# AhmedKishki/AMP-SPARC-SpatialModulation

Hardware: AMD Instinct MI355X
Metric: detected symbol-vectors/sec, VAMP Nt=256 Nr=512 16-QAM; SER match vs ref (higher is better)
Workload: dtype bf16x3; 1 GPU; cfg4: VAMP Nt=256 Nr=512 Na=8 16QAM batch=4096 iterations<=20 EbN0=8.0 dB, one channel per batch; global_batch=4096, parallelism=epoch-shard x1 (independent epochs, one all-reduce of the error counters)

## Files before the change

amp-sparc-spatialmodulation_amd/csrc/amp_denoise.h:

```cpp
#pragma once

#include <float.h>

#include "amp_common.h"

namespace amp {

#define AMP_LOG2E 1.44269504088896340736f

#ifndef AMP_DEN_EXACT_EXP
#define AMP_DEN_EXACT_EXP 0
#endif
#ifndef AMP_DEN_DIV
#define AMP_DEN_DIV 0
#endif
__device__ __forceinline__ float den_exp(float x, float m) {
#if AMP_DEN_EXACT_EXP
    return (float)exp((double)x - (double)m);
#else
    return __builtin_amdgcn_exp2f((x - m) * AMP_LOG2E);
#endif
}
__device__ __forceinline__ float den_rcp(float z) {
#if AMP_DEN_DIV
// ... 542 lines not shown
        for (int i = 0; i < R; ++i) {
            ax = fmaxf(ax, X[i][u]); nx = fminf(nx, X[i][u]);
            ay = fmaxf(ay, Y[i][u]); ny = fminf(ny, Y[i][u]);
        }
        mx[u] = ax; my[u] = ay;
        lmx[u] = ax + ay;
        smax[u] = group_fmax_c<G>(lmx[u]);
        sabs[u] = group_fmax_c<G>(fmaxf(lmx[u], -(nx + ny)));
    }
    const f2v l2e = f2splat(AMP_LOG2E);
#if AMP_DEN_EXACT_EXP
    f2v f = {den_exp(lmx.x, smax.x), den_exp(lmx.y, smax.y)};
#else
    f2v targ = (lmx - smax) * l2e;
    f2v f = {__builtin_amdgcn_exp2f(targ.x), __builtin_amdgcn_exp2f(targ.y)};
#endif
    f2v er[R], ei[R];
#pragma unroll
    for (int i = 0; i < R; ++i) {
#if AMP_DEN_EXACT_EXP
        er[i] = f2v{den_exp(X[i].x, mx.x), den_exp(X[i].y, mx.y)};
        ei[i] = f2v{den_exp(Y[i].x, my.x), den_exp(Y[i].y, my.y)};
#else
        const f2v xa = (X[i] - mx) * l2e, ya = (Y[i] - my) * l2e;
        er[i] = f2v{__builtin_amdgcn_exp2f(xa.x), __builtin_amdgcn_exp2f(xa.y)};
        ei[i] = f2v{__builtin_amdgcn_exp2f(ya.x), __builtin_amdgcn_exp2f(ya.y)};
#endif
    }
    f2v zt, ar, ai, SI = f2splat(0.f);
    f2v Sr[FULLG ? 1 : R];
    if constexpr (FULLG) {
        f2v sr = f2splat(0.f), si = f2splat(0.f), a = f2splat(0.f), b = f2splat(0.f);
#pragma unroll
        for (int i = 0; i < R; ++i) {
            sr += er[i]; si += ei[i];
            a = f2fma(f2splat(Q.re[i]), er[i], a);
            b = f2fma(f2splat(Q.im[i]), ei[i], b);
        }
        SI = si; Sr[0] = sr;
        zt = (sr * si) * f;
        ar = (a * si) * f;
        ai = (sr * b) * f;
    } else {
        f2v z = f2splat(0.f), a = f2splat(0.f), b = f2splat(0.f), w[R];
#pragma unroll
        for (int j = 0; j < R; ++j) w[j] = f2splat(Q.im[j]) * ei[j];
#pragma unroll
        for (int i = 0; i < R; ++i) {
            f2v si = f2splat(0.f), ti = f2splat(0.f);
#pragma unroll
            for (int j = 0; j < R; ++j) {
                const float cw = grid_cnt<PAT>(i, j);
                if (cw == 1.f) { si += ei[j]; ti += w[j]; }
                else if (cw == 2.f) { si = f2fma(f2splat(2.f), ei[j], si); ti = f2fma(f2splat(2.f), w[j], ti); }
            }
            Sr[i] = si;
            const f2v es = er[i] * si;
            z += es;
            a = f2fma(f2splat(Q.re[i]), es, a);
            b = f2fma(er[i], ti, b);
        }
        zt = z * f;
        ar = a * f;
        ai = b * f;
    }
    float ze[2] = {0.f, 0.f}, zt1[2] = {zt.x, zt.y};
#pragma unroll
    for (int u = 0; u < 2; ++u) group_sum_excl_c<G>(zt1[u], ze[u]);
    const f2v iz = {den_rcp(zt1[0]), den_rcp(zt1[1])};
    const f2v xr = ar * iz, xi = ai * iz;
    f2v var = f2splat(0.f);
    if (kVar) {
        f2v vs;
        if constexpr (FULLG) {
            f2v vr = f2splat(0.f), vi = f2splat(0.f);
#pragma unroll
            for (int i = 0; i < R; ++i) {
                const f2v dr = xr - f2splat(Q.re[i]), di = xi - f2splat(Q.im[i]);
                vr = f2fma(dr * dr, er[i], vr);
                vi = f2fma(di * di, ei[i], vi);
            }
            vs = f2fma(vr, SI, Sr[0] * vi) * f;
        } else {
            f2v d[R];
#pragma unroll
            for (int j = 0; j < R; ++j) {
                const f2v di = xi - f2splat(Q.im[j]);
                d[j] = (di * di) * ei[j];
            }
            f2v acc = f2splat(0.f);
#pragma unroll
            for (int i = 0; i < R; ++i) {
                f2v vi = f2splat(0.f);
#pragma unroll
                for (int j = 0; j < R; ++j) {
                    const float cw = grid_cnt<PAT>(i, j);
                    if (cw == 1.f) vi += d[j];
                    else if (cw == 2.f) vi = f2fma(f2splat(2.f), d[j], vi);
                }
                const f2v dr = xr - f2splat(Q.re[i]);
                acc = f2fma(er[i], f2fma(dr * dr, Sr[i], vi), acc);
            }
            vs = acc * f;
        }
        const f2v zev = {ze[0], ze[1]};
        var = (xr * xr + xi * xi) * (zev * iz) + vs * iz;
    }
    xr_out = xr; xi_out = xi; var_out = var; smax_out = smax; sabs_out = sabs;
}

struct Grid2In {
    f2v rr, ri, vp;
};
template <int G, class P>
__device__ __forceinline__ Grid2In grid2_load(const P& pol, int base) {
    const int lane = threadIdx.x & 63;
    constexpr int gpw = 64 / G;
    const int gid = lane / G, g = lane % G;
    Grid2In in;
#pragma unroll
    for (int u = 0; u < 2; ++u) {
        float rr, ri;
        pol.load_r(base + u * gpw + gid, g, rr, ri);
        in.rr[u] = rr; in.ri[u] = ri;
    }
#pragma unroll
    for (int u = 0; u < 2; ++u) in.vp[u] = pol.load_prev(base + u * gpw + gid, g);
    return in;
}
template <bool kVar, int R, int PAT, int G, class P>
__device__ __forceinline__ void denoise_step_grid2_full(const P& pol, int base, const Grid2In& in, const GridRegs<R>& Q,
                                                        PartAcc& pa, DenStat& S) {
    const int lane = threadIdx.x & 63;
    constexpr int gpw = 64 / G;
    const int gid = lane / G, g = lane % G;
    const f2v it = f2splat(pol.inv);
    const f2v ur = in.rr * it, ui = in.ri * it;
    const int bad = (int)!(fabsf(ur.x) <= FLT_MAX) | (int)!(fabsf(ui.x) <= FLT_MAX) | (int)!(fabsf(ur.y) <= FLT_MAX) |
                    (int)!(fabsf(ui.y) <= FLT_MAX);
    S.st_bad |= bad != 0;
    f2v xr, xi, var, smax, sabs;
    grid2_core<kVar, R, PAT, G>(ur, ui, Q, xr, xi, var, smax, sabs);
    pol.store_xv(base + gid, g, xr.x, xi.x, var.x);
    pol.store_xv(base + gpw + gid, g, xr.y, xi.y, var.y);
#pragma unroll
    for (int u = 0; u < 2; ++u) {
        pol.account(var[u], in.vp[u], pa);
        S.st_abs = nan_max(S.st_abs, sabs[u]);
        S.st_min = nan_min(S.st_min, smax[u]);
        pol.section(base + u * gpw + gid, smax[u], sabs[u]);
    }
}

#ifndef AMP_DEN_PACKED_GRID
#define AMP_DEN_PACKED_GRID 1
#endif

template <int KK>
constexpr int grid_r() { return KK == 4 ? 2 : KK == 16 ? 4 : KK == 64 ? 8 : 0; }

template <bool kVar, int KK, int U, int G, bool PKG = true, bool FAST = false, class P>
__device__ __forceinline__ bool denoise_sections_grid(const P& pol, int nsec, const Const& c, PartAcc& pa, DenWaves dw = DenWaves::block()) {
    constexpr int R = grid_r<KK>();
    if constexpr (R == 0) {
        return false;
    } else {
        const int grid = __builtin_amdgcn_readfirstlane(c.grid), gfull = __builtin_amdgcn_readfirstlane(c.gfull);
        if (grid != R) return false;
        const int wave = dw.wave;
        constexpr int gpw = 64 / G;
        const int nw = dw.nw;
        DenStat S;
        GridRegs<R> Q;
        Q.load(c);
        if (gfull == GRID_FULL) {
            for (int base = wave * gpw * U; base < nsec; base += nw * gpw * U) {
                if constexpr (PKG && U == 2 && AMP_DEN_PACKED_GRID)
                    denoise_step_grid2<kVar, R, GRID_FULL, G>(pol, base, nsec, Q, pa, S);
                else
                    denoise_step_grid<kVar, R, GRID_FULL, U, G>(pol, base, nsec, Q, pa, S);
            }
        } else if constexpr (R == 4) {
            int base = wave * gpw * U;
            if constexpr (FAST && PKG && U == 2 && AMP_DEN_PACKED_GRID) {
                const int step = nw * gpw * 2;
                for (; base + 2 * gpw <= nsec; base += step)
                    denoise_step_grid2_full<kVar, R, GRID_REF16, G>(pol, base, grid2_load<G>(pol, base), Q, pa, S);
            }
            for (; base < nsec; base += nw * gpw * U) {
                if constexpr (PKG && U == 2 && AMP_DEN_PACKED_GRID)
                    denoise_step_grid2<kVar, R, GRID_REF16, G>(pol, base, nsec, Q, pa, S);
                else
                    denoise_step_grid<kVar, R, GRID_REF16, U, G>(pol, base, nsec, Q, pa, S);
            }
        }
        S.fold(pa);
        return true;
    }
}

template <bool kVar, int KK, int U, int G, class P>
__device__ __forceinline__ void denoise_sections_gp(const P& pol, int nsec, const Const& c, PartAcc& pa, DenWaves dw = DenWaves::block()) {
    if (denoise_sections_grid<kVar, KK, U, G>(pol, nsec, c, pa, dw)) return;
    const int wave = dw.wave;
    constexpr int gpw = 64 / G;
    const int nw = dw.nw;
    DenRegs<KK> R;
    R.load(c);
    DenStat S;
    for (int base = wave * gpw * U; base < nsec; base += nw * gpw * U)
        denoise_step_gp<kVar, KK, U, G, false>(pol, base, nsec, R, pa, S);
    S.fold(pa);
}

enum { PK_NONE = 0, PK_ALL = 1, PK_GRID = 2 };

template <bool kVar, int KK, int U, int G, int PK, bool FAST = false, class P>
__device__ __forceinline__ void denoise_sections_sel(const P& pol, int nsec, const Const& c, PartAcc& pa, DenWaves dw = DenWaves::block()) {
    if constexpr (PK == PK_ALL && KK % 2 == 0) {
        denoise_sections_gp<kVar, KK, U, G>(pol, nsec, c, pa, dw);
    } else {
        if (denoise_sections_grid<kVar, KK, U, G, PK == PK_GRID, FAST>(pol, nsec, c, pa, dw)) return;
        denoise_sections_g<kVar, KK, U, G>(pol, nsec, c, pa, dw);
    }
}
template <bool kVar, int KK, int U, int PK = PK_ALL, bool FAST = false, class P>
__device__ __forceinline__ void denoise_sections_u(const P& pol, int nsec, int M, const Const& c, PartAcc& pa, DenWaves dw = DenWaves::block()) {
    switch (M) {
    case 64: denoise_sections_sel<kVar, KK, U, 64, PK, FAST>(pol, nsec, c, pa, dw); break;
    case 32: denoise_sections_sel<kVar, KK, U, 32, PK, FAST>(pol, nsec, c, pa, dw); break;
    case 16: denoise_sections_sel<kVar, KK, U, 16, PK, FAST>(pol, nsec, c, pa, dw); break;
    case 8: denoise_sections_sel<kVar, KK, U, 8, PK, FAST>(pol, nsec, c, pa, dw); break;
    case 4: denoise_sections_sel<kVar, KK, U, 4, PK, FAST>(pol, nsec, c, pa, dw); break;
    case 2: denoise_sections_sel<kVar, KK, U, 2, PK, FAST>(pol, nsec, c, pa, dw); break;
    default: denoise_sections_sel<kVar, KK, U, 1, PK, FAST>(pol, nsec, c, pa, dw); break;
    }
}

template <bool kVar, int KK, int G, class P>
__device__ __forceinline__ void denoise_sections_wide(const P& pol, int nsec, const Const& c, PartAcc& pa, DenWaves dw = DenWaves::block()) {
    static_assert(KK % 8 == 0, "chunks of 8 points");
    if (denoise_sections_grid<kVar, KK, 1, G>(pol, nsec, c, pa, dw)) return;
    const int lane = threadIdx.x & 63, wave = dw.wave;
    constexpr int gpw = 64 / G;
    const int gid = lane / G, g = lane % G;
    const int nw = dw.nw;
    __shared__ float s_cre[KK], s_cim[KK];
    __syncthreads();
    if (threadIdx.x == 0) {
#pragma unroll
        for (int k = 0; k < KK; ++k) { s_cre[k] = kval(c.re[k]); s_cim[k] = kval(c.im[k]); }
    }
    __syncthreads();
    DenStat S;
    for (int base = wave * gpw; base < nsec; base += nw * gpw) {
        const int sec = base + gid;
        const bool act = sec < nsec;
        float rr, ri, it;
        pol.load(act ? sec : nsec - 1, g, rr, ri, it);
        const float ur = rr * it, ui = ri * it;
        if (act) S.st_bad |= !(fabsf(ur) <= FLT_MAX && fabsf(ui) <= FLT_MAX);
        float lmax = -FLT_MAX, lmin = FLT_MAX;
#pragma unroll 1
        for (int k0 = 0; k0 < KK; k0 += 8) {
#pragma unroll
            for (int j = 0; j < 8; ++j) {
                const float x = fmaf(ur, s_cre[k0 + j], ui * s_cim[k0 + j]);
                lmax = fmaxf(lmax, x);
                lmin = fminf(lmin, x);
            }
        }
        const float smax = group_fmax_c<G>(lmax), sabs = group_fmax_c<G>(fmaxf(lmax, -lmin));
        float zm = 0.f, a = 0.f, b = 0.f;
#pragma unroll 1
        for (int k0 = 0; k0 < KK; k0 += 8) {
#pragma unroll
            for (int j = 0; j < 8; ++j) {
                const float cr = s_cre[k0 + j], ci = s_cim[k0 + j];
                const float e = den_exp(fmaf(ur, cr, ui * ci), smax);
                zm += e;
                a = fmaf(cr, e, a);
                b = fmaf(ci, e, b);
            }
        }
        float zt = zm, ze = 0.f;
        group_sum_excl_c<G>(zt, ze);
        const float iz = den_rcp(zt);
        const float xr = a * iz, xi = b * iz;
        float var = 0.f;
        if (kVar) {
            float vs = 0.f;
#pragma unroll 1
            for (int k0 = 0; k0 < KK; k0 += 8) {
#pragma unroll
                for (int j = 0; j < 8; ++j) {
                    const float cr = s_cre[k0 + j], ci = s_cim[k0 + j];
                    const float e = den_exp(fmaf(ur, cr, ui * ci), smax);
                    const float dr = xr - cr, di = xi - ci;
                    vs = fmaf(fmaf(dr, dr, di * di), e, vs);
                }
            }
            var = (xr * xr + xi * xi) * (ze * iz) + vs * iz;
        }
        if (act) {
            pol.store(sec, g, xr, xi, var, pa);
            S.st_abs = nan_max(S.st_abs, sabs);
            S.st_min = nan_min(S.st_min, smax);
            if (g == 0) pol.section(sec, smax, sabs);
        }
    }
    S.fold(pa);
}

template <bool kVar, int KK, class P>
__device__ __forceinline__ void denoise_sections_wide_m(const P& pol, int nsec, int M, const Const& c, PartAcc& pa, DenWaves dw = DenWaves::block()) {
    switch (M) {
    case 64: denoise_sections_wide<kVar, KK, 64>(pol, nsec, c, pa, dw); break;
    case 32: denoise_sections_wide<kVar, KK, 32>(pol, nsec, c, pa, dw); break;
    case 16: denoise_sections_wide<kVar, KK, 16>(pol, nsec, c, pa, dw); break;
    case 8: denoise_sections_wide<kVar, KK, 8>(pol, nsec, c, pa, dw); break;
    case 4: denoise_sections_wide<kVar, KK, 4>(pol, nsec, c, pa, dw); break;
    case 2: denoise_sections_wide<kVar, KK, 2>(pol, nsec, c, pa, dw); break;
    default: denoise_sections_wide<kVar, KK, 1>(pol, nsec, c, pa, dw); break;
    }
}

template <bool kVar, int KK, class P>
__device__ __forceinline__ void denoise_sections(const P& pol, int nsec, int M, const Const& c, PartAcc& pa) {
    if constexpr (KK > 16) {
        denoise_sections_wide_m<kVar, KK>(pol, nsec, M, c, pa);
        return;
    } else {
    if (M <= 64) {
        denoise_sections_u<kVar, KK, 1>(pol, nsec, M, c, pa);
        return;
    }
    const int lane = threadIdx.x & 63, wave = threadIdx.x >> 6;
    const int G = M < 64 ? M : 64;
    const int PPL = M / G;
    const int gpw = 64 / G;
    const int gid = lane / G, g = lane - gid * G;
    const int nw = blockDim.x >> 6;
    for (int base = wave * gpw; base < nsec; base += nw * gpw) {
        const int sec = base + gid;
        const bool act = sec < nsec;
        const int ss = act ? sec : nsec - 1;
        float lmax = -FLT_MAX, lmin = FLT_MAX;
        bool bad = false;
        {
            for (int p = 0; p < PPL; ++p) {
                float rr, ri, it;
                pol.load(ss, g + p * 64, rr, ri, it);
                const float ur = rr * it, ui = ri * it;
                bad |= !(fabsf(ur) <= FLT_MAX && fabsf(ui) <= FLT_MAX);
#pragma unroll
                for (int k = 0; k < KK; ++k) {
                    {
                        const float x = fmaf(ur, c.re[k], ui * c.im[k]);
                        lmax = fmaxf(lmax, x);
                        lmin = fminf(lmin, x);
                    }
                }
            }
            const float smax = group_fmax(lmax, 64);
            double zl = 0.0;
            for (int p = 0; p < PPL; ++p) {
                float rr, ri, it;
                pol.load(ss, g + p * 64, rr, ri, it);
                const float ur = rr * it, ui = ri * it;
                float zm = 0.f;
#pragma unroll
                for (int k = 0; k < KK; ++k)
                    zm += __builtin_amdgcn_exp2f((fmaf(ur, c.re[k], ui * c.im[k]) - smax) * AMP_LOG2E);
                zl += (double)zm;
            }
            const double z = group_sum(zl, 64);
            const double iz = 1.0 / z;
            for (int p = 0; p < PPL; ++p) {
                float rr, ri, it;
// ... 131 lines not shown
```

amp-sparc-spatialmodulation_amd/csrc/amp_vamp.h:

```cpp
#pragma once

#include "amp_decide.h"
#include "amp_denoise.h"
#include "amp_gemm.h"
#include "amp_host.h"

namespace amp {

constexpr int RWG = 1024;
constexpr int PBAR_EPOCH = 64;
constexpr int PBAR_WORDS = PBAR_EPOCH + 256;

struct VampK {
    int B, N, n, k, L, M;
    int Bmean;
    int kap0, ncp0, kap1, ncp1, kap2, ncp2, bn2;
    int nblk2, max_iter;
    double noise_var, sparsity;
    const float* Wt0;
    const float* Wt1;
    const float* Wt2;
    const float* s;
    float* s2;
    float* ytil;
// ... 141 lines not shown
    }
    ss = group_sum(ss, 64);
    const float varL = (float)(ss / (double)P.k) * (float)P.noise_var;
    const double eta = (double)P.k / (double)P.N;
    float xtv, s2t32;
    if (first) {
        xtv = (float)eta * varL + (float)((1.0 - eta) * s2t64);
        s2t32 = (float)s2t64;
    } else {
        xtv = (float)eta * varL + (float)(1.0 - eta) * s2t;
        s2t32 = s2t;
    }
    const float alpha = clampf_t(xtv / s2t32, AMP_VAR_RATIO_MIN, 1.0f - AMP_VAR_RATIO_MIN);
    const float sigma2 = clampf_t((alpha / (1.0f - alpha)) * s2t32, AMP_VAR_MIN, AMP_VAR_MAX);
    it.vr = vr;
    it.alpha = alpha;
    it.inv1ma = 1.0f / (1.0f - alpha);
    it.sigma2 = sigma2;
    it.inv_sigma2 = 1.0f / sigma2;
    it.s2t = s2t32;
}

__device__ inline VampIter vamp_first_iter(const VampK& P, float* lds, const S2Lane* sl = nullptr) {
    VampIter it;
    it.stopped = 0; it.T = 0; it.fixed = 0; it.fixed_all = 0; it.G = 0.0;
    it.pad1[0] = it.pad1[1] = it.pad1[2] = 0.f;
    it.dxdr_prev = 0.f;
    it.ns_prev = 1.f;
    const double p = P.sparsity;
    vamp_lmmse_scalars(P, true, p * p * (1 - p) + (1 - p) * (1 - p) * p, 0.f, lds, it, sl);
    return it;
}

__device__ inline VampIter vamp_advance(const VampK& P, const VampIter& cur, const PartAcc& pa, int fixed, int t,
                                        float* lds, const S2Lane* sl = nullptr) {
    VampIter nx;
    nx.stopped = 0; nx.T = 0; nx.fixed = fixed; nx.fixed_all = (fixed < 0) ? 1 : 0; nx.G = pa.maxabs;
    nx.pad1[0] = nx.pad1[1] = nx.pad1[2] = 0.f;
    if (pa.notclose == 0) {
        nx = cur;
        nx.stopped = 1;
        nx.T = t + 1;
        nx.fixed = fixed;
    } else {
        const float mean = (float)(pa.sumvar / ((double)P.Bmean * (double)P.N));
        const float dxdr = clampf_t(mean / cur.sigma2, AMP_VAR_RATIO_MIN, 1.0f - AMP_VAR_RATIO_MIN);
        const float ns = 1.0f / (1.0f - dxdr);
        const float s2t = clampf_t((cur.sigma2 * dxdr) * ns, AMP_VAR_MIN, AMP_VAR_MAX);
        nx.dxdr_prev = dxdr;
        nx.ns_prev = ns;
        vamp_lmmse_scalars(P, false, 0.0, s2t, lds, nx, sl);
    }
    return nx;
}

__device__ inline VampIter vamp_advance_head(const VampK& P, const VampIter& cur, const PartAcc& pa, int fixed, int t) {
    VampIter nx;
    nx.stopped = 0; nx.T = 0; nx.fixed = fixed; nx.fixed_all = (fixed < 0) ? 1 : 0; nx.G = pa.maxabs;
    nx.pad1[0] = nx.pad1[1] = nx.pad1[2] = 0.f;
    nx.vr = nx.alpha = nx.inv1ma = nx.sigma2 = nx.inv_sigma2 = 0.f;
    if (pa.notclose == 0) {
        nx = cur;
        nx.stopped = 1;
        nx.T = t + 1;
        nx.fixed = fixed;
    } else {
        const float mean = (float)(pa.sumvar / ((double)P.Bmean * (double)P.N));
        const float dxdr = clampf_t(mean / cur.sigma2, AMP_VAR_RATIO_MIN, 1.0f - AMP_VAR_RATIO_MIN);
        const float ns = 1.0f / (1.0f - dxdr);
        nx.dxdr_prev = dxdr;
        nx.ns_prev = ns;
        nx.s2t = clampf_t((cur.sigma2 * dxdr) * ns, AMP_VAR_MIN, AMP_VAR_MAX);
    }
    return nx;
}

__device__ inline void vamp_advance_tail(const VampK& P, VampIter& it, const S2Lane& sl) {
    const float s2t = it.s2t;
    const float vr = (1.0f / s2t) * (float)P.noise_var;
    const int lane = threadIdx.x & 63;
    float q[4];
#pragma unroll
    for (int j = 0; j < 4; ++j) q[j] = 1.0f / (sl.v[j] + vr);
    double ss = 0.0;
#pragma unroll
    for (int j = 0; j < 4; ++j) ss += (lane + 64 * j < P.k) ? (double)q[j] : 0.0;
    ss = group_sum(ss, 64);
    const float varL = (float)(ss / (double)P.k) * (float)P.noise_var;
    const float xtv = P.etaf * varL + P.ometaf * s2t;
    const float alpha = clampf_t(xtv / s2t, AMP_VAR_RATIO_MIN, 1.0f - AMP_VAR_RATIO_MIN);
    const float sigma2 = clampf_t((alpha / (1.0f - alpha)) * s2t, AMP_VAR_MIN, AMP_VAR_MAX);
    it.vr = vr;
    it.alpha = alpha;
    it.inv1ma = 1.0f / (1.0f - alpha);
    it.sigma2 = sigma2;
    it.inv_sigma2 = 1.0f / sigma2;
}

__device__ inline amp_status vamp_make_status(const VampK& P, const VampIter& cur, const VampIter& nx, int fixed) {
    amp_status s;
    s.T = nx.stopped ? nx.T : P.max_iter;
    s.nan_state = fixed != 0 ? 1 : 0;
    s.stopped = nx.stopped;
    s.gemm = P.x3 + 1;
    s.last_scalar[0] = cur.s2t; s.last_scalar[1] = cur.alpha; s.last_scalar[2] = cur.sigma2;
    s.last_scalar[3] = nx.stopped ? cur.dxdr_prev : nx.dxdr_prev;
    return s;
}

struct PDenoisePolicy {
    const float* r;
    float* x;
    float* vnew;
    const float* vprev;
    float* sm;
    float* sa;
    int ldr, M, lspr, N;
    float inv;
    __device__ __forceinline__ void load(int sec, int m, float& rr, float& ri, float& it) const {
        const int row = sec >> lspr, sj = sec & ((1 << lspr) - 1);
        const float2 v = *reinterpret_cast<const float2*>(r + row * ldr + 2 * (sj * M + m));
        rr = v.x; ri = v.y; it = inv;
    }
    __device__ __forceinline__ void store(int sec, int m, float xr, float xi, float var, PartAcc& pa) const {
        const int row = sec >> lspr, sj = sec & ((1 << lspr) - 1);
        *reinterpret_cast<float2*>(x + row * ldr + 2 * (sj * M + m)) = make_float2(xr, xi);
        const int vo = row * N + sj * M + m;
        vnew[vo] = var;
        pa.sumvar += (double)var;
        pa.notclose += torch_close(var, vprev[vo]) ? 0u : 1u;
    }
    __device__ __forceinline__ void section(int sec, float smax, float sabs) const {
        sm[sec] = smax;
        sa[sec] = sabs;
    }
    __device__ __forceinline__ void load_r(int sec, int m, float& rr, float& ri) const {
        const int row = sec >> lspr, sj = sec & ((1 << lspr) - 1);
        const float2 v = *reinterpret_cast<const float2*>(r + row * ldr + 2 * (sj * M + m));
        rr = v.x; ri = v.y;
    }
    __device__ __forceinline__ float load_prev(int sec, int m) const {
        const int row = sec >> lspr, sj = sec & ((1 << lspr) - 1);
        return vprev[row * N + sj * M + m];
    }
    __device__ __forceinline__ void store_xv(int sec, int m, float xr, float xi, float var) const {
        const int row = sec >> lspr, sj = sec & ((1 << lspr) - 1);
        *reinterpret_cast<float2*>(x + row * ldr + 2 * (sj * M + m)) = make_float2(xr, xi);
        vnew[row * N + sj * M + m] = var;
    }
    __device__ __forceinline__ void account(float var, float vp, PartAcc& pa) const {
        pa.sumvar += (double)var;
        pa.notclose += torch_close(var, vp) ? 0u : 1u;
    }
    float* dbg = nullptr;
};
__device__ __forceinline__ void den_debug(const PDenoisePolicy& p, int sec, int m, float ze, float vs) {
    if (p.dbg) {
        const int row = sec >> p.lspr, sj = sec & ((1 << p.lspr) - 1);
        p.dbg[row * 2 * p.N + sj * p.M + m] = ze;
        p.dbg[row * 2 * p.N + p.N + sj * p.M + m] = vs;
    }
}

constexpr int PBM = 16;

bool vamp_persist_eligible(const amp_dims* d, int k, int ncu, int epochs = 1, int gemm = AMP_GEMM_AUTO);
int vamp_persist_max_epochs(const amp_dims* d, int k, int ncu, int gemm = AMP_GEMM_AUTO);
int vamp_persist_wg_per_cu(const amp_dims* d, int k, int gemm);
int vamp_gemm_select(const amp_dims* d, int k, int gemm);
bool vamp_persist_x3_fits(int N, int k, int L, int K = 0);
bool vamp_persist_ytil_in_kernel(const VampK& P);
bool vamp_persist_ytil_h2(const VampK& P);
int vamp_persist_launch(const VampK& P, const Const64& c64, const DecConst& dc, hipStream_t st, int ncu);
int device_cu_count();
float* debug_dump_ptr();
bool gemm_f32_requested();
bool persist_wg2();

}
```

amp-sparc-spatialmodulation_amd/csrc/amp_vamp_persist.hip:

```cpp
#include <stdlib.h>

#include <algorithm>
#include <mutex>
#include <vector>

#include "amp_vamp_persist_kernel.h"

namespace amp {

__global__ __launch_bounds__(1024) void vamp_decide_fold(const DecWG* w, int n, amp_counts* out) {
    __shared__ DecWG s[16];
    dec_fold_block(w + (size_t)blockIdx.x * n, n, out + blockIdx.x, s);
}

static std::once_flag g_pers_once;
static int g_ncu = 0;

int device_cu_count() {
    std::call_once(g_pers_once, [] {
        int dev = 0;
        if (hipGetDevice(&dev) != hipSuccess || hipDeviceGetAttribute(&g_ncu, hipDeviceAttributeMultiprocessorCount,
                                                                      dev) != hipSuccess)
            g_ncu = 0;
    });
    return g_ncu;
}

bool vamp_persist_ytil_in_kernel(const VampK& P) {
    return P.n == 2 * P.N && PBM * (2 * P.n + 4) <= playout(P.N, P.k, P.L).offV0;
}

bool vamp_persist_ytil_h2(const VampK& P) {
    return P.n == 2 * P.N && P.k == P.N && 2 * PBM * pl_ldx(P.n) <= playout(P.N, P.k, P.L, true).offV0;
}

bool vamp_persist_x3_fits(int N, int k, int L, int K) {
    const size_t fixed = K > 16 ? 5120 : 2048;
    return k == N && N % 64 == 0 && (size_t)playout(N, k, L, true).total * 4 + fixed <= 160 * 1024;
}

bool persist_wg2() {
    static const bool v = [] {
        const char* e = diag_env("AMP_PERSIST_WG2");
        return !(e && e[0] == '0') && !gemm_f32_requested();
    }();
    return v;
}
static bool persist_pair_epochs() {
    static const bool v = [] {
        const char* e = diag_env("AMP_EPOCHS_TWO_PER_CU");
        return e && e[0] == '1';
    }();
    return v;
}
static int persist_wg_cap(int N, int gemm_mode) {
    return (N == 64 && (gemm_mode == 1 || gemm_mode == 2) && persist_wg2() && persist_pair_epochs()) ? 2 : 1;
}

int vamp_persist_wg_per_cu(const amp_dims* d, int k, int gemm) {
    return persist_wg_cap(d->N, vamp_gemm_select(d, k, gemm));
}

int vamp_persist_max_epochs(const amp_dims* d, int k, int ncu, int gemm) {
    const int gemm_mode = vamp_gemm_select(d, k, gemm);
    if (!vamp_persist_shape(d, k) || d->n % 2 != 0 || d->M > 64) return 0;
    if ((size_t)playout(d->N, k, d->L).total * 4 + 2048 > 160 * 1024) return 0;
    const int wpe = cdiv(d->B, PBM);
    if (wpe > ncu) return 0;
    if (d->B % PBM != 0) return 1;
    return std::max(1, persist_wg_cap(d->N, gemm_mode) * ncu / wpe);
}

bool vamp_persist_eligible(const amp_dims* d, int k, int ncu, int epochs, int gemm) {
    if (!vamp_persist_shape(d, k) || d->n % 2 != 0 || d->M > 64) return false;
    if (epochs < 1 || (epochs > 1 && d->B % PBM != 0)) return false;
    if (cdiv(d->B, PBM) > ncu ||
        (long)epochs * cdiv(d->B, PBM) > (long)persist_wg_cap(d->N, vamp_gemm_select(d, k, gemm)) * ncu)
        return false;
    return (size_t)playout(d->N, k, d->L).total * 4 + 2048 <= 160 * 1024;
}

static int persist_dispatch(const VampK& P, const DecConst& dc, hipStream_t st);
int persist_dispatch_x3(const VampK& P, const DecConst& dc, hipStream_t st);
int persist_dispatch_h2(const VampK& P, const DecConst& dc, hipStream_t st);
int persist_dispatch_i8(const VampK& P, const DecConst& dc, hipStream_t st);

static std::mutex g_tm_mu;
static bool g_tm_on = false;
static std::vector<std::pair<hipEvent_t, hipEvent_t>> g_tm_ev;

int vamp_persist_launch(const VampK& P, const Const64& c64, const DecConst& dc, hipStream_t st, int ncu) {
    (void)ncu;
    DecConst d2 = dc;
    static_cast<Const64&>(d2) = c64;
    hipEvent_t te[2] = {nullptr, nullptr};
    {
        std::lock_guard<std::mutex> lk(g_tm_mu);
        if (g_tm_on && hipEventCreate(&te[0]) == hipSuccess && hipEventCreate(&te[1]) == hipSuccess) {
            g_tm_ev.emplace_back(te[0], te[1]);
            (void)hipEventRecord(te[0], st);
        } else {
            te[0] = te[1] = nullptr;
        }
    }
    const int rc = persist_dispatch(P, d2, st);
    if (te[1]) (void)hipEventRecord(te[1], st);
    if (rc || !P.dec_on || P.fold_in) return rc;
    hipLaunchKernelGGL(vamp_decide_fold, dim3(P.E), dim3(256), 0, st, (const DecWG*)P.dwg, P.nwg / P.E, P.counts);
    AMP_LAUNCH_CHECK("vamp_decide_fold");
    return AMP_OK;
}

static int persist_dispatch(const VampK& P, const DecConst& dc, hipStream_t st) {
    if (P.x3 == 3) return persist_dispatch_i8(P, dc, st);
    if (P.x3 == 2) return persist_dispatch_h2(P, dc, st);
    if (P.x3) return persist_dispatch_x3(P, dc, st);
    switch (P.N) {
    case 64: return persist_launch_nt<2, 4, false>(P, dc, st);
    case 128: return persist_launch_nt<4, 4, false>(P, dc, st);
    case 256: return persist_launch_nt<8, 4, false>(P, dc, st);
    default: break;
    }
    set_error("vamp_persist: N = %d not supported", P.N);
    return AMP_E_ARG;
}

}

int amp_debug_persist_timing(int32_t on) {
    std::lock_guard<std::mutex> lk(amp::g_tm_mu);
    amp::g_tm_on = on != 0;
    return AMP_OK;
}

int amp_debug_persist_time(int32_t* n, float* mean_ms) {
    AMP_REQUIRE(n && mean_ms, "amp_debug_persist_time: null output");
    std::lock_guard<std::mutex> lk(amp::g_tm_mu);
    double tot = 0.0;
    int cnt = 0;
    for (auto& e : amp::g_tm_ev) {
        float ms = 0.f;
        if (hipEventSynchronize(e.second) == hipSuccess && hipEventElapsedTime(&ms, e.first, e.second) == hipSuccess) {
            tot += ms;
            ++cnt;
        }
        (void)hipEventDestroy(e.first);
        (void)hipEventDestroy(e.second);
    }
    amp::g_tm_ev.clear();
    *n = cnt;
    *mean_ms = cnt ? (float)(tot / cnt) : 0.f;
    return AMP_OK;
}
```

amp-sparc-spatialmodulation_amd/csrc/amp_vamp_persist_kernel.h:

```cpp
#pragma once

#include <stdlib.h>

#include <type_traits>

#include "amp_decide_fused.h"
#include "amp_persist.h"
#include "amp_vamp.h"

namespace amp {

constexpr int AMP_TRACE_STRIDE = 10;
#ifndef AMP_OCC2_PK
#define AMP_OCC2_PK 0
#endif
#ifndef AMP_KK4_DU
#define AMP_KK4_DU 4
#endif
#ifndef AMP_X3_W8_PIN
#define AMP_X3_W8_PIN 0
#endif
#ifndef AMP_X3_W8_RING
#define AMP_X3_W8_RING 1
#endif
#ifndef AMP_X3_W8_PKGRID
#define AMP_X3_W8_PKGRID 1
#endif
#ifndef AMP_X3_W8_DENFAST
#define AMP_X3_W8_DENFAST 1
#endif
#ifndef AMP_DECIDE_NARROW
#define AMP_DECIDE_NARROW 1
#endif
#ifndef AMP_X3_DU
#define AMP_X3_DU 2
#endif
#ifndef AMP_SCALAR_TAIL
#define AMP_SCALAR_TAIL 1
#endif

struct PLayout {
    int lda, ldr;
    int offA, offR, offX, offV0, offV1, offSM, offSA, offScr, total;
};

__host__ __device__ inline int x3_ldx(int N) { return pl_ldx(N); }
__host__ __device__ inline int x3_plane_floats(int N) { return 6 * 16 * x3_ldx(N) / 2; }

__host__ __device__ inline PLayout playout(int N, int k, int L, bool x3 = false) {
    PLayout y;
    y.lda = (2 * N > 2 * k ? 2 * N : 2 * k) + 4;
    y.ldr = 2 * N + (x3 ? 8 : 4);
    int o = 0;
    y.offA = o; o += (x3 && x3_plane_floats(N) > PBM * y.lda) ? x3_plane_floats(N) : PBM * y.lda;
    y.offR = o; o += PBM * y.ldr;
    y.offX = o; o += PBM * y.ldr;
    y.offV0 = o; o += PBM * N;
    y.offV1 = o; o += PBM * N;
    y.offSM = o; o += PBM * L;
    y.offSA = o; o += PBM * L;
    o = (o + 3) & ~3;
    y.offScr = o; o += 1024;
    y.total = o;
    return y;
}

constexpr int KARG_DC_OFF = karg_second_offset<VampK, DecConst>();

template <int NT, int KK, int NWV, int DU, bool X3, int OCC = 1, bool H2 = false, bool I8 = false>
__global__ __launch_bounds__(64 * NWV, OCC * NWV / 4) void vamp_persist(VampK P_arg, DecConst dc_arg) {
    (void)P_arg;
    (void)dc_arg;
    unsigned long long kbase = karg_base();
    const VampK* Pp = karg_at<VampK>(kbase, 0);
    const DecConst* Dp = karg_at<DecConst>(kbase, KARG_DC_OFF);
#define P (*Pp)
#define dc (*Dp)
    static_assert(!X3 || ((NWV == 4 || (NWV == 8 && !H2 && OCC == 1)) && NT % 2 == 0),
                  "X3: four waves (eight for the bf16x3 two-waves-per-SIMD form), whole complex tiles");
    static_assert(!(H2 && I8) && (!I8 || X3), "I8: a split-precision form of its own");
    constexpr int PKDEN = ((OCC * NWV / 4 == 1) || AMP_OCC2_PK) ? PK_ALL
                          : (NWV == 8 && KK == 16 && AMP_X3_W8_PKGRID) ? PK_GRID : PK_NONE;
    constexpr bool DENFAST = NWV == 8 && OCC == 1 && PKDEN == PK_GRID && AMP_X3_W8_DENFAST;
    constexpr int PWG = 64 * NWV;
    constexpr int NC = X3 ? NT / 2 : 1;
    constexpr int G3 = NT * NWV / 4;
    constexpr int X3R = (NWV == 8) ? AMP_X3_W8_RING : 1;
    constexpr bool X3PIN = NWV == 8 && AMP_X3_W8_PIN;
    constexpr bool X3PF = X3 && !H2 && !I8;
    constexpr int PFT = (NC + 1) / 2;
    constexpr int STAIL = (X3PF && OCC == 1) ? AMP_SCALAR_TAIL : 0;
#define c64 (static_cast<const Const64&>(*Dp))
    extern __shared__ __attribute__((aligned(16))) float lds[];
    __shared__ int s_flag;
    __shared__ double s_d[PWG / 64][4];
    __shared__ float s_hmax[PWG / 64][PBM];
    __shared__ int s_hexp[PBM];
    __shared__ float s_s2[STAIL != 0 ? 256 : 1];
    const PLayout Y = playout(P.N, P.k, P.L, X3);
    float* sA = lds + Y.offA;
    float* sR = lds + Y.offR;
    float* sX = lds + Y.offX;
    float* sM = lds + Y.offSM;
    float* sS = lds + Y.offSA;
    float* scr = lds + Y.offScr;
    const int tid = threadIdx.x, lane = tid & 63, wave = tid >> 6;
    const int wg = blockIdx.x, nwg = gridDim.x;
    const int wgx = wg + P.wg_off, nwx = P.nwg_x;
    const int ep = wgx / P.wpe, wl = wgx - ep * P.wpe, wg0 = ep * P.wpe;
    const int lrow0 = wl * PBM;
    const int row0 = ep * P.B + lrow0 - P.row_off, nrows = min(PBM, P.B - lrow0);
#define ebar (P.pbar + (P.E > 1 ? PBAR_EPOCH + ep : 0))
    const int N = P.N, twoN = 2 * N, twok = 2 * P.k, M = P.M, spr = N / M;
    const float* const sv_ep = P.s + (size_t)ep * P.sch;
#define Wx1 ((const void*)((const char*)P.Wx1 + ep * P.wch))
#define Wx2 ((const void*)((const char*)P.Wx2 + ep * P.wch))
    const int ldr = Y.ldr, lda = Y.lda;
    const int ct0 = wave * NT;
    const int cc0 = wave * NC;
    unsigned short* sP = reinterpret_cast<unsigned short*>(sA);
    const int ldx = x3_ldx(N);
    signed char* sB = reinterpret_cast<signed char*>(sA);
    const int ldb = i8_ldb(N);

    float yt[NT][4], s2c[NT];
#pragma unroll
    for (int t = 0; t < NT; ++t) {
        const int col = X3 ? 2 * (16 * (cc0 + (t < NC ? t : 0)) + (lane & 15)) : 16 * (ct0 + t) + (lane & 15);
        const float sv = sv_ep[col >> 1];
        s2c[t] = sv * sv;
    }
    if (H2 && P.ytil_in_kernel) {
      if constexpr (H2) {
        constexpr int IPY = NT / 2;
        const int n = P.n, ldy = pl_ldx(n);
        const int row = tid % PBM;
        float re[IPY][8], im[IPY][8];
        float m = 0.f;
#pragma unroll
        for (int i = 0; i < IPY; ++i) {
            const int e = tid + i * PWG;
            const int j0 = 8 * (e / PBM);
#pragma unroll
            for (int h = 0; h < 4; ++h) {
                float4 v = *reinterpret_cast<const float4*>(P.y + (size_t)(row0 + max(min(row, nrows - 1), 0)) * 2 * n + 2 * j0 + 4 * h);
                if (!(row < nrows)) v = make_float4(0.f, 0.f, 0.f, 0.f);
                re[i][2 * h] = v.x; im[i][2 * h] = v.y; re[i][2 * h + 1] = v.z; im[i][2 * h + 1] = v.w;
            }
#pragma unroll
            for (int h = 0; h < 8; ++h) m = fmaxf(m, fmaxf(fabsf(re[i][h]), fabsf(im[i][h])));
        }
        m = fmaxf(m, __shfl_xor(m, 16));
        m = fmaxf(m, __shfl_xor(m, 32));
        if (lane < PBM) s_hmax[wave][lane] = m;
        __syncthreads();
        float mr = s_hmax[0][row];
#pragma unroll
        for (int w = 1; w < PWG / 64; ++w) mr = fmaxf(mr, s_hmax[w][row]);
        const int ex = h2_row_exp(mr);
        if (tid < PBM) s_hexp[tid] = ex;
#pragma unroll
        for (int i = 0; i < IPY; ++i) {
            const int e = tid + i * PWG;
#pragma unroll
            for (int h = 0; h < 8; ++h) {
                re[i][h] = __builtin_amdgcn_ldexpf(re[i][h], ex);
                im[i][h] = __builtin_amdgcn_ldexpf(im[i][h], ex);
            }
            h2_store8(sP, ldy, row, 8 * (e / PBM), re[i], im[i]);
        }
        __syncthreads();
        f32x4 yr[NC], yi[NC];
        gemm_h2<NC, 2 * G3>(sP, ldy, P.Wq0, cc0, yr, yi);
#pragma unroll
        for (int r = 0; r < 4; ++r) {
            const float sc = __builtin_amdgcn_ldexpf(1.0f, -(s_hexp[4 * (lane >> 4) + r] + YH2_EX));
#pragma unroll
            for (int t = 0; t < NC; ++t) {
                yt[2 * t][r] = yr[t][r] * sc;
                yt[2 * t + 1][r] = yi[t][r] * sc;
            }
        }
        __syncthreads();
      }
    } else if (X3) {
      if constexpr (!I8) {
#pragma unroll
        for (int t = 0; t < NC; ++t) {
            const int o = 16 * (cc0 + t) + (lane & 15);
#pragma unroll
            for (int r = 0; r < 4; ++r) {
                const int row = 4 * (lane >> 4) + r;
                const bool in = row < nrows;
                const size_t yo = (size_t)(row0 + max(min(row, nrows - 1), 0)) * twok + 2 * o;
                const float a = P.ytil[yo], b = P.ytil[yo + 1];
                yt[2 * t][r] = in ? a : 0.f;
                yt[2 * t + 1][r] = in ? b : 0.f;
            }
        }
      }
    } else if (P.ytil_in_kernel) {
        const int ldy = 4 * N + 4;
        for (int e = tid; e < PBM * N; e += PWG) {
            const int row = e / N, c4 = 4 * (e - row * N);
            float4 v = *reinterpret_cast<const float4*>(P.y + (size_t)(row0 + max(min(row, nrows - 1), 0)) * 4 * N + c4);
            if (!(row < nrows)) v = make_float4(0.f, 0.f, 0.f, 0.f);
            *reinterpret_cast<float4*>(lds + row * ldy + c4) = v;
        }
        __syncthreads();
        f32x4 acc[NT];
        gemm16<NT, 2 * NT * NWV>(lds, ldy, P.Wq0, ct0, acc);
#pragma unroll
        for (int t = 0; t < NT; ++t)
#pragma unroll
            for (int r = 0; r < 4; ++r) yt[t][r] = acc[t][r];
        __syncthreads();
    } else {
#pragma unroll
        for (int t = 0; t < NT; ++t) {
            const int col = 16 * (ct0 + t) + (lane & 15);
#pragma unroll
            for (int r = 0; r < 4; ++r) {
                const int row = 4 * (lane >> 4) + r;
                const float yv = P.ytil[(size_t)(row0 + max(min(row, nrows - 1), 0)) * twok + col];
                yt[t][r] = (row < nrows) ? yv : 0.f;
            }
        }
    }
    VampIter cur;
    {
        const S2Lane s2l = s2_lane(P, sv_ep);
        cur = vamp_first_iter(P, scr, &s2l);
        if constexpr (STAIL != 0) {
            if (wave == 0) {
#pragma unroll
                for (int j = 0; j < 4; ++j) s_s2[lane + 64 * j] = s2l.v[j];
// ... 553 lines not shown
```

Baseline: 6.084 million symbol-vectors/s.

## Add paired-lane grid denoise path with vectorized loads/stores for 16-QAM

Adds a new denoiser fast path for the 16-QAM grid case with G=32 and eight waves. Each lane now handles two adjacent symbols of one section, so r/x can be read and written as float4 and the variances as float2, and the per-section max reduction needs fewer cross-lane steps. The variance sum is carried in a lane-permuted double accumulator using permlane32_swap and bpermute, so the reduction order matches the old per-lane layout. A host check is added that rejects LDS layouts whose rows are not 16-byte aligned. The risks are extra permute instructions and possible small changes in floating-point ordering.

```diff
diff --git a/amp-sparc-spatialmodulation_amd/csrc/amp_denoise.h b/amp-sparc-spatialmodulation_amd/csrc/amp_denoise.h
--- a/amp-sparc-spatialmodulation_amd/csrc/amp_denoise.h
+++ b/amp-sparc-spatialmodulation_amd/csrc/amp_denoise.h
@@ -718,14 +718,212 @@
     }
 }
 
+template <bool kVar, int R, int PAT>
+__device__ __forceinline__ void grid2_pair_core(const f2v ur, const f2v ui, const GridRegs<R>& Q, f2v& xr_out, f2v& xi_out,
+                                                f2v& var_out, float& smax_out, float& sabs_out) {
+    constexpr bool FULLG = PAT == GRID_FULL;
+    f2v X[R], Y[R];
+#pragma unroll
+    for (int i = 0; i < R; ++i) {
+        X[i] = ur * f2splat(Q.re[i]);
+        Y[i] = ui * f2splat(Q.im[i]);
+    }
+    f2v mx, my, lmx, lab;
+#pragma unroll
+    for (int u = 0; u < 2; ++u) {
+        float ax = -FLT_MAX, nx = FLT_MAX, ay = -FLT_MAX, ny = FLT_MAX;
+#pragma unroll
+        for (int i = 0; i < R; ++i) {
+            ax = fmaxf(ax, X[i][u]); nx = fminf(nx, X[i][u]);
+            ay = fmaxf(ay, Y[i][u]); ny = fminf(ny, Y[i][u]);
+        }
+        mx[u] = ax; my[u] = ay;
+        lmx[u] = ax + ay;
+        lab[u] = fmaxf(lmx[u], -(nx + ny));
+    }
+    int kmax = max(fkey(lmx.x), fkey(lmx.y)), kabs = max(fkey(lab.x), fkey(lab.y));
+    kmax = imax_step<1>(kmax); kabs = imax_step<1>(kabs);
+    kmax = imax_step<2>(kmax); kabs = imax_step<2>(kabs);
+    kmax = imax_step<4>(kmax); kabs = imax_step<4>(kabs);
+    kmax = imax_step<8>(kmax); kabs = imax_step<8>(kabs);
+    const float smax1 = funkey(kmax), sabs1 = funkey(kabs);
+    const f2v smax = f2splat(smax1);
+    const f2v l2e = f2splat(AMP_LOG2E);
+#if AMP_DEN_EXACT_EXP
+    f2v f = {den_exp(lmx.x, smax.x), den_exp(lmx.y, smax.y)};
+#else
+    f2v targ = (lmx - smax) * l2e;
+    f2v f = {__builtin_amdgcn_exp2f(targ.x), __builtin_amdgcn_exp2f(targ.y)};
+#endif
+    f2v er[R], ei[R];
+#pragma unroll
+    for (int i = 0; i < R; ++i) {
+#if AMP_DEN_EXACT_EXP
+        er[i] = f2v{den_exp(X[i].x, mx.x), den_exp(X[i].y, mx.y)};
+        ei[i] = f2v{den_exp(Y[i].x, my.x), den_exp(Y[i].y, my.y)};
+#else
+        const f2v xa = (X[i] - mx) * l2e, ya = (Y[i] - my) * l2e;
+        er[i] = f2v{__builtin_amdgcn_exp2f(xa.x), __builtin_amdgcn_exp2f(xa.y)};
+        ei[i] = f2v{__builtin_amdgcn_exp2f(ya.x), __builtin_amdgcn_exp2f(ya.y)};
+#endif
+    }
+    f2v zt, ar, ai, SI = f2splat(0.f);
+    f2v Sr[FULLG ? 1 : R];
+    if constexpr (FULLG) {
+        f2v sr = f2splat(0.f), si = f2splat(0.f), a = f2splat(0.f), b = f2splat(0.f);
+#pragma unroll
+        for (int i = 0; i < R; ++i) {
+            sr += er[i]; si += ei[i];
+            a = f2fma(f2splat(Q.re[i]), er[i], a);
+            b = f2fma(f2splat(Q.im[i]), ei[i], b);
+        }
+        SI = si; Sr[0] = sr;
+        zt = (sr * si) * f;
+        ar = (a * si) * f;
+        ai = (sr * b) * f;
+    } else {
+        f2v z = f2splat(0.f), a = f2splat(0.f), b = f2splat(0.f), w[R];
+#pragma unroll
+        for (int j = 0; j < R; ++j) w[j] = f2splat(Q.im[j]) * ei[j];
+#pragma unroll
+        for (int i = 0; i < R; ++i) {
+            f2v si = f2splat(0.f), ti = f2splat(0.f);
+#pragma unroll
+            for (int j = 0; j < R; ++j) {
+                const float cw = grid_cnt<PAT>(i, j);
+                if (cw == 1.f) { si += ei[j]; ti += w[j]; }
+                else if (cw == 2.f) { si = f2fma(f2splat(2.f), ei[j], si); ti = f2fma(f2splat(2.f), w[j], ti); }
+            }
+            Sr[i] = si;
+            const f2v es = er[i] * si;
+            z += es;
+            a = f2fma(f2splat(Q.re[i]), es, a);
+            b = f2fma(er[i], ti, b);
+        }
+        zt = z * f;
+        ar = a * f;
+        ai = b * f;
+    }
+    float tot = zt.x + zt.y;
+    f2v zev = {0.f + zt.y, 0.f + zt.x};
+    {
+        float p = xl<1>(tot);
+        zev.x += p; zev.y += p; tot = tot + p;
+        p = xl<2>(tot);
+        zev.x += p; zev.y += p; tot = tot + p;
+        p = xl<4>(tot);
+        zev.x += p; zev.y += p; tot = tot + p;
+        p = xl<8>(tot);
+        zev.x += p; zev.y += p; tot = tot + p;
+    }
+    const f2v iz = f2splat(den_rcp(tot));
+    const f2v xr = ar * iz, xi = ai * iz;
+    f2v var = f2splat(0.f);
+    if (kVar) {
+        f2v vs;
+        if constexpr (FULLG) {
+            f2v vr = f2splat(0.f), vi = f2splat(0.f);
+#pragma unroll
+            for (int i = 0; i < R; ++i) {
+                const f2v dr = xr - f2splat(Q.re[i]), di = xi - f2splat(Q.im[i]);
+                vr = f2fma(dr * dr, er[i], vr);
+                vi = f2fma(di * di, ei[i], vi);
+            }
+            vs = f2fma(vr, SI, Sr[0] * vi) * f;
+        } else {
+            f2v d[R];
+#pragma unroll
+            for (int j = 0; j < R; ++j) {
+                const f2v di = xi - f2splat(Q.im[j]);
+                d[j] = (di * di) * ei[j];
+            }
+            f2v acc = f2splat(0.f);
+#pragma unroll
+            for (int i = 0; i < R; ++i) {
+                f2v vi = f2splat(0.f);
+#pragma unroll
+                for (int j = 0; j < R; ++j) {
+                    const float cw = grid_cnt<PAT>(i, j);
+                    if (cw == 1.f) vi += d[j];
+                    else if (cw == 2.f) vi = f2fma(f2splat(2.f), d[j], vi);
+                }
+                const f2v dr = xr - f2splat(Q.re[i]);
+                acc = f2fma(er[i], f2fma(dr * dr, Sr[i], vi), acc);
+            }
+            vs = acc * f;
+        }
+        var = (xr * xr + xi * xi) * (zev * iz) + vs * iz;
+    }
+    xr_out = xr; xi_out = xi; var_out = var; smax_out = smax1; sabs_out = sabs1;
+}
+
+__device__ __forceinline__ double pair_acc_move(double v, int src_lane) {
+    const long long b = __double_as_longlong(v);
+    const int lo = __builtin_amdgcn_ds_bpermute(4 * src_lane, (int)(unsigned)b);
+    const int hi = __builtin_amdgcn_ds_bpermute(4 * src_lane, (int)(b >> 32));
+    return __longlong_as_double((long long)(((unsigned long long)(unsigned)hi << 32) | (unsigned)lo));
+}
+__device__ __forceinline__ int pair_lane() {
+    int l = threadIdx.x & 63;
+    asm volatile("" : "+v"(l));
+    return l;
+}
+__device__ __forceinline__ double pair_acc_in(double sumvar) {
+    const int n = pair_lane();
+    return pair_acc_move(sumvar, ((n >> 4) & 1) * 32 + 2 * (n & 15) + (n >> 5));
+}
+__device__ __forceinline__ double pair_acc_out(double acc) {
+    const int l = pair_lane();
+    return pair_acc_move(acc, (l & 1) * 32 + (l >> 5) * 16 + ((l & 31) >> 1));
+}
+
+struct GridPairIn {
+    f2v rr, ri, vp;
+};
+template <class P>
+__device__ __forceinline__ GridPairIn grid2_pair_load(const P& pol, int base, int lane) {
+    const int sec = base + (lane >> 4), m = 2 * (lane & 15);
+    GridPairIn in;
+    const float4 v = pol.load_r2(sec, m);
+    const float2 p = pol.load_prev2(sec, m);
+    in.rr = f2v{v.x, v.z}; in.ri = f2v{v.y, v.w};
+    in.vp = f2v{p.x, p.y};
+    asm volatile("" : "+v"(in.vp));
+    return in;
+}
+template <bool kVar, int R, int PAT, class P>
+__device__ __forceinline__ void denoise_step_grid2_pair(const P& pol, int base, int lane, const GridPairIn& in,
+                                                        const GridRegs<R>& Q, PartAcc& pa, double& acc, DenStat& S) {
+    const int sec = base + (lane >> 4), m = 2 * (lane & 15);
+    const f2v it = f2splat(pol.inv);
+    const f2v ur = in.rr * it, ui = in.ri * it;
+    const int bad = (int)!(fabsf(ur.x) <= FLT_MAX) | (int)!(fabsf(ui.x) <= FLT_MAX) | (int)!(fabsf(ur.y) <= FLT_MAX) |
+                    (int)!(fabsf(ui.y) <= FLT_MAX);
+    S.st_bad |= bad != 0;
+    f2v xr, xi, var;
+    float smax, sabs;
+    grid2_pair_core<kVar, R, PAT>(ur, ui, Q, xr, xi, var, smax, sabs);
+    pol.store_xv2(sec, m, make_float4(xr.x, xi.x, xr.y, xi.y), make_float2(var.x, var.y));
+    const auto sw = __builtin_amdgcn_permlane32_swap(__float_as_uint(var.x), __float_as_uint(var.y), false, false);
+    acc += (double)__uint_as_float(sw[0]);
+    acc += (double)__uint_as_float(sw[1]);
+    pol.account_close(var.x, in.vp.x, pa);
+    pol.account_close(var.y, in.vp.y, pa);
+    S.st_abs = nan_max(S.st_abs, sabs);
+    S.st_min = nan_min(S.st_min, smax);
+    pol.section(sec, smax, sabs);
+}
+
 #ifndef AMP_DEN_PACKED_GRID
 #define AMP_DEN_PACKED_GRID 1
 #endif
 
+enum { DEN_FAST_NONE = 0, DEN_FAST_FULL = 1, DEN_FAST_PAIR = 2 };
+
 template <int KK>
 constexpr int grid_r() { return KK == 4 ? 2 : KK == 16 ? 4 : KK == 64 ? 8 : 0; }
 
-template <bool kVar, int KK, int U, int G, bool PKG = true, bool FAST = false, class P>
+template <bool kVar, int KK, int U, int G, bool PKG = true, int FAST = DEN_FAST_NONE, class P>
 __device__ __forceinline__ bool denoise_sections_grid(const P& pol, int nsec, const Const& c, PartAcc& pa, DenWaves dw = DenWaves::block()) {
     constexpr int R = grid_r<KK>();
     if constexpr (R == 0) {
@@ -750,8 +948,19 @@
             int base = wave * gpw * U;
             if constexpr (FAST && PKG && U == 2 && AMP_DEN_PACKED_GRID) {
                 const int step = nw * gpw * 2;
-                for (; base + 2 * gpw <= nsec; base += step)
-                    denoise_step_grid2_full<kVar, R, GRID_REF16, G>(pol, base, grid2_load<G>(pol, base), Q, pa, S);
+                if constexpr (FAST == DEN_FAST_PAIR && G == 32) {
+                    base = __builtin_amdgcn_readfirstlane(base);
+                    double acc = pair_acc_in(pa.sumvar);
+                    for (; base + 2 * gpw <= nsec; base += step) {
+                        const int lane = pair_lane();
+                        denoise_step_grid2_pair<kVar, R, GRID_REF16>(pol, base, lane, grid2_pair_load(pol, base, lane), Q, pa,
+                                                                     acc, S);
+                    }
+                    pa.sumvar = pair_acc_out(acc);
+                } else {
+                    for (; base + 2 * gpw <= nsec; base += step)
+                        denoise_step_grid2_full<kVar, R, GRID_REF16, G>(pol, base, grid2_load<G>(pol, base), Q, pa, S);
+                }
             }
             for (; base < nsec; base += nw * gpw * U) {
                 if constexpr (PKG && U == 2 && AMP_DEN_PACKED_GRID)
@@ -781,7 +990,7 @@
 
 enum { PK_NONE = 0, PK_ALL = 1, PK_GRID = 2 };
 
-template <bool kVar, int KK, int U, int G, int PK, bool FAST = false, class P>
+template <bool kVar, int KK, int U, int G, int PK, int FAST = DEN_FAST_NONE, class P>
 __device__ __forceinline__ void denoise_sections_sel(const P& pol, int nsec, const Const& c, PartAcc& pa, DenWaves dw = DenWaves::block()) {
     if constexpr (PK == PK_ALL && KK % 2 == 0) {
         denoise_sections_gp<kVar, KK, U, G>(pol, nsec, c, pa, dw);
@@ -790,7 +999,7 @@
         denoise_sections_g<kVar, KK, U, G>(pol, nsec, c, pa, dw);
     }
 }
-template <bool kVar, int KK, int U, int PK = PK_ALL, bool FAST = false, class P>
+template <bool kVar, int KK, int U, int PK = PK_ALL, int FAST = DEN_FAST_NONE, class P>
 __device__ __forceinline__ void denoise_sections_u(const P& pol, int nsec, int M, const Const& c, PartAcc& pa, DenWaves dw = DenWaves::block()) {
     switch (M) {
     case 64: denoise_sections_sel<kVar, KK, U, 64, PK, FAST>(pol, nsec, c, pa, dw); break;
diff --git a/amp-sparc-spatialmodulation_amd/csrc/amp_vamp.h b/amp-sparc-spatialmodulation_amd/csrc/amp_vamp.h
--- a/amp-sparc-spatialmodulation_amd/csrc/amp_vamp.h
+++ b/amp-sparc-spatialmodulation_amd/csrc/amp_vamp.h
@@ -317,6 +317,22 @@
         pa.sumvar += (double)var;
         pa.notclose += torch_close(var, vp) ? 0u : 1u;
     }
+    __device__ __forceinline__ float4 load_r2(int sec, int m) const {
+        const int row = sec >> lspr, sj = sec & ((1 << lspr) - 1);
+        return *reinterpret_cast<const float4*>(r + row * ldr + 2 * (sj * M + m));
+    }
+    __device__ __forceinline__ float2 load_prev2(int sec, int m) const {
+        const int row = sec >> lspr, sj = sec & ((1 << lspr) - 1);
+        return *reinterpret_cast<const float2*>(vprev + row * N + sj * M + m);
+    }
+    __device__ __forceinline__ void store_xv2(int sec, int m, float4 xv, float2 var) const {
+        const int row = sec >> lspr, sj = sec & ((1 << lspr) - 1);
+        *reinterpret_cast<float4*>(x + row * ldr + 2 * (sj * M + m)) = xv;
+        *reinterpret_cast<float2*>(vnew + row * N + sj * M + m) = var;
+    }
+    __device__ __forceinline__ void account_close(float var, float vp, PartAcc& pa) const {
+        pa.notclose += torch_close(var, vp) ? 0u : 1u;
+    }
     float* dbg = nullptr;
 };
 __device__ __forceinline__ void den_debug(const PDenoisePolicy& p, int sec, int m, float ze, float vs) {
diff --git a/amp-sparc-spatialmodulation_amd/csrc/amp_vamp_persist.hip b/amp-sparc-spatialmodulation_amd/csrc/amp_vamp_persist.hip
--- a/amp-sparc-spatialmodulation_amd/csrc/amp_vamp_persist.hip
+++ b/amp-sparc-spatialmodulation_amd/csrc/amp_vamp_persist.hip
@@ -91,6 +91,13 @@
 
 int vamp_persist_launch(const VampK& P, const Const64& c64, const DecConst& dc, hipStream_t st, int ncu) {
     (void)ncu;
+    if (P.x3) {
+        const PLayout y = playout(P.N, P.k, P.L, true);
+        if ((y.ldr | P.N | y.offR | y.offX | y.offV0 | y.offV1) % 4 != 0) {
+            set_error("vamp_persist: LDS rows not 16-byte aligned (N = %d, ldr = %d)", P.N, y.ldr);
+            return AMP_E_ARG;
+        }
+    }
     DecConst d2 = dc;
     static_cast<Const64&>(d2) = c64;
     hipEvent_t te[2] = {nullptr, nullptr};
diff --git a/amp-sparc-spatialmodulation_amd/csrc/amp_vamp_persist_kernel.h b/amp-sparc-spatialmodulation_amd/csrc/amp_vamp_persist_kernel.h
--- a/amp-sparc-spatialmodulation_amd/csrc/amp_vamp_persist_kernel.h
+++ b/amp-sparc-spatialmodulation_amd/csrc/amp_vamp_persist_kernel.h
@@ -28,6 +28,9 @@
 #endif
 #ifndef AMP_X3_W8_DENFAST
 #define AMP_X3_W8_DENFAST 1
+#endif
+#ifndef AMP_X3_W8_DENPAIR
+#define AMP_X3_W8_DENPAIR 1
 #endif
 #ifndef AMP_DECIDE_NARROW
 #define AMP_DECIDE_NARROW 1
@@ -81,7 +84,8 @@
     static_assert(!(H2 && I8) && (!I8 || X3), "I8: a split-precision form of its own");
     constexpr int PKDEN = ((OCC * NWV / 4 == 1) || AMP_OCC2_PK) ? PK_ALL
                           : (NWV == 8 && KK == 16 && AMP_X3_W8_PKGRID) ? PK_GRID : PK_NONE;
-    constexpr bool DENFAST = NWV == 8 && OCC == 1 && PKDEN == PK_GRID && AMP_X3_W8_DENFAST;
+    constexpr int DENFAST = !(NWV == 8 && OCC == 1 && PKDEN == PK_GRID && AMP_X3_W8_DENFAST) ? DEN_FAST_NONE
+                            : AMP_X3_W8_DENPAIR ? DEN_FAST_PAIR : DEN_FAST_FULL;
     constexpr int PWG = 64 * NWV;
     constexpr int NC = X3 ? NT / 2 : 1;
     constexpr int G3 = NT * NWV / 4;
```

Result: faster. 6.207 million symbol-vectors/s, median of 6 (+2.0%).
